# qcc4cp/qcc

Hardware: AMD Instinct MI355X
Metric: gate-applies/sec (2^30-amplitude units), QFT (higher is better)
Workload: dtype f64; 1 GPU; 30-qubit QFT complex128, 465 gates/step (qc.qft order), basis-state input, state resident in HBM, 2^30 amplitudes per GPU [BASELINE config 2]; qubits=30, fusion=1

## Files before the change

include/qcc_hip.h:

```cpp
#ifndef QCC_HIP_H_
#define QCC_HIP_H_

#include <stdint.h>

#ifdef __cplusplus
extern "C" {
#endif

typedef struct qh_state_s *qh_handle;

#define QH_OK 0
#define QH_ERR_BAD_QUBIT 1
#define QH_ERR_SAME_QUBIT 2
#define QH_ERR_BAD_DTYPE 3
#define QH_ERR_HIP 4
#define QH_ERR_ARG 5
#define QH_ERR_NOMEM 6
#define QH_ERR_NO_DEVICE 7
#define QH_ERR_NONLOCAL 8
#define QH_ERR_COMM 9

#define QH_FUSE_OFF 0
#define QH_FUSE_SWEEP 1

// ... 80 lines not shown
int qh_comm_destroy(qh_handle h);
int qh_exchange_alltoall(qh_handle h, int base_bit, uint64_t chunk_amps);
int qh_exchange_pair(qh_handle h, int shard_bit, int local_bit, uint64_t chunk_amps);
int qh_exchange_loopback(qh_handle h, int local_bit, uint64_t chunk_amps);
int qh_exchange_wait(qh_handle h);
int qh_exchange_stats(qh_handle h, qh_xstats *out);
int qh_comm_allreduce_sum(qh_handle h, double *inout, int count);

int qh_norm2(qh_handle h, double *out);
int qh_amplitude(qh_handle h, uint64_t logical_index, double out[2]);
int qh_argmax(qh_handle h, uint64_t *phys_index, double *prob);
int qh_prob_bit(qh_handle h, int logical_bit, double *p1);
int qh_prob_bit_value(qh_handle h, int logical_bit, int value, double *p);
int qh_scale(qh_handle h, double re, double im);
int qh_project_bit(qh_handle h, int logical_bit, int value);
int qh_marginal(qh_handle h, int k, const int32_t *bits, double *out);
int qh_sample(qh_handle h, uint64_t count, const double *u, uint64_t *logical_out);
int qh_project_bits(qh_handle h, uint64_t mask, uint64_t value);
int qh_expect_pauli(qh_handle h, uint64_t nterms, const uint64_t *xmask, const uint64_t *zmask, double *out);
typedef struct { uint64_t index; double re, im; } qh_entry;
#define QH_SELECT_MAX (1u << 20)
#define QH_TOPK_MAX 4096
int qh_select(qh_handle h, double threshold, uint64_t cap, qh_entry *out, uint64_t *count, double *weight);
int qh_topk(qh_handle h, uint64_t k, qh_entry *out, uint64_t *count);
int qh_amplitudes(qh_handle h, uint64_t count, const uint64_t *logical, double *out, uint64_t *nlocal);

int qh_clone(qh_handle src, qh_handle *out);
int qh_copy(qh_handle dst, qh_handle src);
int qh_inner(qh_handle a, qh_handle b, double out[2]);
#define QH_INNER_LINEAR 0
#define QH_INNER_TILES 1
#define QH_INNER_GATHER 2
typedef struct {
  uint32_t path;
  uint32_t nrest;
  uint64_t free_a, free_b;
  uint8_t tile_a[8], tile_b[8], shuffle[8];
  uint8_t rest_a[56], rest_b[56];
  uint8_t pos_b[64];
} qh_inner_tiles;
int qh_inner_plan(qh_handle a, qh_handle b, qh_inner_tiles *out);
int qh_axpby(qh_handle dst, const double alpha[2], qh_handle src, const double beta[2], double *norm2);

int qh_extend(qh_handle src, int k, const double *amps, uint64_t basis, qh_handle *out);
int qh_release(qh_handle src, int k, const int32_t *bits, uint64_t value, double weight[2], qh_handle *out);

typedef struct {
  uint64_t gates_submitted;
  uint64_t kernels_launched;
  uint64_t sweeps;
  uint64_t bytes_algorithmic;
  uint64_t bytes_swept;
  uint64_t gates_noop;
} qh_stats;
int qh_get_stats(qh_handle h, qh_stats *out);
int qh_reset_stats(qh_handle h);
int qh_timer_begin(qh_handle h);
int qh_timer_end(qh_handle h, float *milliseconds);
int qh_timer_lap(qh_handle h);
int qh_timer_laps(qh_handle h, float *milliseconds, int cap, int *count);
int qh_plan_json(qh_handle h, char *buf, uint64_t cap, uint64_t *needed);

int qh_plan_export(qh_handle h, void *buf, uint64_t cap, uint64_t *needed);

int qh_plan_handlers(qh_handle h, void *buf, uint64_t cap, uint64_t *needed);

int qh_host_apply1(void *psi, const double gate[8], int nbits, int tgt,
                   int bit_width);
int qh_host_applyc(void *psi, const double gate[8], int nbits, int ctl, int tgt,
                   int bit_width);
int qh_host_release(void);

#ifdef __cplusplus
}
#endif
#endif
```

qcc_amd/csrc/engine.hip:

```cpp
#include <hip/hip_runtime.h>

#include <algorithm>
#include <chrono>
#include <cmath>
#include <cstdarg>
#include <cstddef>
#include <cstdio>
#include <cstdlib>
#include <cstring>
#include <ctime>
#include <string>
#include <vector>

#include "../../include/qcc_hip.h"
#include "buffers.hip.h"
#include "kernels_gate.hip.h"
#include "kernels_dense.hip.h"
#include "kernels_mux.hip.h"
#include "kernels_measure.hip.h"
#include "kernels_select.hip.h"
#include "select_plan.h"
#include "kernels_expect.hip.h"
#include "kernels_inner.hip.h"
#include "kernels_axpby.hip.h"
// ... 2393 lines not shown
                    (uint32_t)__builtin_popcountll(xmask[t] & zmask[t]) & 3u};
  }
  std::stable_sort(terms.begin(), terms.end(), [](const Term &l, const Term &r) { return l.px < r.px; });
  qh::ScratchLayout lay;
  const size_t slab_off = lay.add((size_t)kExpectBlocks * qh::kExpectT * sizeof(double)), out_off = lay.add((size_t)nterms * sizeof(double));
  HIP_TRY(h->meas.reserve(lay.total));
  double *slab = (double *)(h->meas.as<char>() + slab_off), *dout = (double *)(h->meas.as<char>() + out_off);
  uint64_t batches = 0;
  for (uint64_t first = 0; first < nterms;) {
    uint64_t cnt = 1;
    while (first + cnt < nterms && cnt < (uint64_t)qh::kExpectT && terms[first + cnt].px == terms[first].px) ++cnt;
    const uint64_t px = terms[first].px;
    const bool pair = (px >> 6) != 0;
    qh::ExpectArgs a{};
    a.x = px;
    a.tb = pair ? 63 - __builtin_clzll(px) : 0;
    const int per_bits = pair ? 3 : 4, nom = 8 + per_bits, wbits = pair ? h->nloc - 1 : h->nloc;
    a.cw = std::min(nom, wbits);
    const uint64_t nchunks = 1ull << (wbits - a.cw), nblk = std::min(nchunks, kExpectBlocks);
    a.cpb = (uint32_t)(nchunks / nblk);
    for (uint64_t k = 0; k < cnt; ++k) {
      const Term &tm = terms[first + k];
      uint64_t z = tm.pz;
      if (pair) z = (z & ((1ull << a.tb) - 1ull)) | ((z >> (a.tb + 1)) << a.tb);
      a.zt[k] = (uint8_t)(z & 255ull);
      const uint32_t zu = (uint32_t)(z >> 8) & ((1u << per_bits) - 1u);
      for (uint32_t u = 0; u < (1u << per_bits); ++u) a.zu[k] |= (uint16_t)((__builtin_popcount(u & zu) & 1) << u);
      a.zc[k] = z >> nom;
      const uint32_t one = (((tm.ny >> 1) ^ tm.neg) & 1u) ? 0xBFF00000u : 0x3FF00000u;
      if (tm.ny & 1u) a.cim[k] = one; else a.cre[k] = one;
    }
    const int tt = cnt <= 4 ? 4 : qh::kExpectT;
    with_real(h, [&](auto x) {
      using R = decltype(x);
      if (tt == 4) launch_expect<R, 4>(h, pair, (unsigned)nblk, a, slab);
      else launch_expect<R, qh::kExpectT>(h, pair, (unsigned)nblk, a, slab);
    });
    hipLaunchKernelGGL(qh::k_expect_fold, dim3((unsigned)cnt), dim3(256), 0, h->stream, (const double *)slab, (uint32_t)nblk, tt,
                       pair ? 2.0 : 1.0, dout + first);
    if ((rc = check_launch(h))) return rc;
    first += cnt;
    ++batches;
  }
  std::vector<double> vals(nterms);
  if ((rc = read_back(h, vals.data(), dout, (size_t)nterms * sizeof(double)))) return rc;
  for (uint64_t k = 0; k < nterms; ++k) out[terms[k].idx] = vals[k];
  h->stats.kernels_launched += batches;
  h->stats.bytes_swept += batches * ((1ull << h->nloc) * h->amp_bytes());
  return QH_OK;
}

int qh_get_stats(qh_handle h, qh_stats *out) {
  if (!h || !out) return fail(QH_ERR_ARG, "null");
  *out = h->stats;
  return QH_OK;
}
int qh_reset_stats(qh_handle h) {
  if (!h) return fail(QH_ERR_ARG, "null");
  h->stats = qh_stats{};
  return QH_OK;
}

int qh_timer_begin(qh_handle h) {
  if (!h) return fail(QH_ERR_ARG, "null handle");
  int rc = enter(h);
  if (rc) return rc;
  rc = make_events(h);
  if (rc) return rc;
  HIP_TRY(hipEventRecord(h->ev0, h->stream));
  return QH_OK;
}
int qh_timer_end(qh_handle h, float *ms) {
  if (!h || !ms) return fail(QH_ERR_ARG, "null handle or out");
  if (!h->ev0) return fail(QH_ERR_ARG, "qh_timer_end without qh_timer_begin");
  int rc = enter(h);
  if (rc) return rc;
  HIP_TRY(hipEventRecord(h->ev1, h->stream));
  if ((rc = wait_event(h, h->ev1, "qh_timer_end"))) return rc;
  HIP_TRY(hipEventElapsedTime(ms, h->ev0, h->ev1));
  return QH_OK;
}

int qh_timer_lap(qh_handle h) {
  if (!h) return fail(QH_ERR_ARG, "null handle");
  const int rc = enter(h);
  if (rc) return rc;
  if (h->laps_used == h->laps.size()) {
    hipEvent_t e = nullptr;
    HIP_TRY(hipEventCreate(&e));
    h->laps.push_back(e);
  }
  HIP_TRY(hipEventRecord(h->laps[h->laps_used++], h->stream));
  return QH_OK;
}
int qh_timer_laps(qh_handle h, float *ms, int cap, int *count) {
  if (!h || !count || h->dry) return fail(QH_ERR_ARG, "null/dry");
  HIP_TRY(hipSetDevice(h->device));
  const int n = h->laps_used > 0 ? (int)h->laps_used - 1 : 0;
  if (h->laps_used) {
    const int rc = wait_event(h, h->laps[h->laps_used - 1], "qh_timer_laps");
    if (rc) return rc;
  }
  for (int k = 0; k < n && ms && k < cap; ++k) HIP_TRY(hipEventElapsedTime(&ms[k], h->laps[k], h->laps[k + 1]));
  *count = n;
  h->laps_used = 0;
  return QH_OK;
// ... 647 lines not shown
```

qcc_amd/csrc/kernels_sweep.hip.h:

```cpp
#pragma once
#include <hip/hip_runtime.h>

#include <string>
#include <vector>

#include "kernels_gate.hip.h"
#include <deque>
#include <memory>

#include "planner.h"
#include "exchange.hip.h"

namespace qh {

struct SweepParams {
  const SweepOp *ops;
  const DGroup *groups;
  const OTerm *oterms;
  uint32_t nops;
  uint32_t tables_rel;
  uint32_t n_ltab_lds;
  uint32_t pad0;
  uint64_t store_delta_mask;
  uint64_t prof_buf;
  uint64_t tilemax;
  uint64_t slot_off[64];
  uint64_t slot_off_store[64];
};
static_assert(kMaxInsertBits + kMaxSlabBits <= kMaxIns, "planner/kernels disagree on inserted bits");
static_assert(kExchangeSlabBits == kMaxSlabBits, "exchange_plan.h / planner disagree on slab bits");
static_assert(sizeof(SweepOp) == 96 && sizeof(DGroup) == 64 && sizeof(OTerm) == 24, "asm island layouts");
static_assert(offsetof(SweepParams, slot_off) == 0x40 && offsetof(SweepParams, nops) == 0x18 && offsetof(SweepParams, tilemax) == 0x38 &&
                  offsetof(SweepParams, slot_off_store) == 0x240 && offsetof(SweepParams, store_delta_mask) == 0x28,
              "asm island layouts");

struct LaneGeom {
  int lane_low;
  int rot;
  int blk_bits;
  int nwave;
  int wpos[kMaxWaveBits];
  int wdst[kMaxWaveBits];
  int ltab_in_island;
};

constexpr uint64_t kProfRows = 8192, kProfRecs = 128;
struct UnitPerm {
  int n;
  int shift[kMaxUnitSegs];
  uint64_t mask[kMaxUnitSegs];
  int nslab;
  int slab_pos[kMaxSlabBits];
  uint64_t slab_val;
};

struct alignas(8) SweepArgs {
  uint64_t psi;
  uint64_t dst;
  uint64_t prm;
  uint64_t idx_high;
  uint64_t nunits;
  uint64_t ins_ones;
  uint64_t slab_val;
  uint64_t ltab_src;
  uint32_t n_ltab;
  uint32_t exch_bytes;
  uint32_t stride_units;
  uint32_t seat_dest;
  uint8_t ins_n, lane_low, rot, blk_bits;
  uint8_t nwave, wpos[2], island_copies;
  uint8_t wdst[2], up_n, up_nslab;
  uint8_t slab_pos[kMaxSlabBits], wpb;
  uint8_t seat[8];
  uint8_t ins_pos[16];
  int8_t up_shift[kMaxUnitSegs];
  uint64_t up_mask[kMaxUnitSegs];
};
static_assert(kMaxUnitSegs == 8 && kMaxSlabBits == 3 && kMaxIns <= 16 && kMaxWaveBits == 2 && kLaneBits <= 8, "SweepArgs layout");
static_assert(offsetof(SweepArgs, n_ltab) == 64 && offsetof(SweepArgs, ins_n) == 80 && offsetof(SweepArgs, ins_pos) == 104 &&
                  offsetof(SweepArgs, up_shift) == 120 && offsetof(SweepArgs, up_mask) == 128 && sizeof(SweepArgs) == 192,
              "SweepArgs layout (k_sweep reads it by dword index)");

typedef uint32_t qh_u32x16 __attribute__((ext_vector_type(16)));

inline int flush_pace(const PlanResult &pr, bool wide, int nloc) {
  if (const char *e = getenv("QH_SWEEP_PACE")) return atoi(e);
  if (!wide || pr.sweeps.empty()) return 0;
  double joules = 0, ms = 0;
  for (const SweepPlan &sp : pr.sweeps) {
    if (sp.nwave > 1) return 0;
    const double units = (double)sp.swept_bytes / (2.0 * 16.0 * (double)(1ull << 30));
    ms += (nloc <= 31 ? 5.45 : 5.85) * units;
    joules += 4.9 * units + sweep_op_energy_nj(sp) * (double)sp.ntiles * 1e-9 * 1.15;
  }
  const double watts = joules / ms * 1e3;
  return (watts >= 1320.0 && watts <= 1450.0) ? 12 : 0;
}

template <int RB, bool WIDE>
__global__ __launch_bounds__(256) void k_sweep(SweepArgs args_in_kernarg_segment) {
  constexpr uint32_t kAmp = WIDE ? 16u : 8u;
#ifdef QH_PROF
  const uint64_t prof_t_entry = __builtin_amdgcn_s_memtime();
#endif
  const uint32_t lane_u = threadIdx.x & 63;
  const uint32_t wave_s = __builtin_amdgcn_readfirstlane(threadIdx.x >> 6);
  extern __shared__ __attribute__((aligned(16))) unsigned char xbuf[];
  const uint32_t lds_base = (uint32_t)(uintptr_t)(__attribute__((address_space(3))) unsigned char *)xbuf;
  for (uint32_t turn = 0;; ++turn) {
    qh_u32x16 q0, q1, q2;
    asm volatile("s_load_dwordx16 %0, %3, 0x0\n\ts_load_dwordx16 %1, %3, 0x40\n\ts_load_dwordx16 %2, %3, 0x80\n\t"
                 "s_waitcnt lgkmcnt(0)"
                 : "=&s"(q0), "=&s"(q1), "=&s"(q2)
                 : "s"((uint64_t)(uintptr_t)__builtin_amdgcn_kernarg_segment_ptr()));
    auto dw = [&](int i) -> uint32_t { return i < 16 ? q0[i] : i < 32 ? q1[i - 16] : q2[i - 32]; };
    auto qw = [&](int i) -> uint64_t { return (uint64_t)dw(i) | ((uint64_t)dw(i + 1) << 32); };
    auto by = [&](int i, int b) -> uint32_t { return (dw(i) >> (8 * b)) & 255u; };
    const uint32_t lane_low = by(20, 1), nwave = by(21, 0), wpb = by(23, 3);
    const uint32_t n_lt = dw(16), exch_bytes = dw(17);
    const uint32_t lds_ltab = lds_base + exch_bytes;
    const uint32_t wg_threads = wpb << 6;
    const bool island_copies = by(21, 3) != 0;
    if (turn == 0 && n_lt && !island_copies) {
      typedef double v2d_t __attribute__((ext_vector_type(2)));
      const __attribute__((address_space(1))) v2d_t *src = (const __attribute__((address_space(1))) v2d_t *)qw(14);
      v2d_t *dst = (v2d_t *)(xbuf + exch_bytes);
      for (uint32_t i = threadIdx.x; i < n_lt * 64u; i += wg_threads) dst[i] = src[i];
      __syncthreads();
    }
    const uint32_t nlt_now = island_copies && turn == 0 ? n_lt : 0u;
    uint64_t bi = blockIdx.x;
    const uint32_t rot = by(20, 2), blk_bits = by(20, 3);
    if (rot) bi = ((bi >> rot) | (bi << (blk_bits - rot))) & ((1ull << blk_bits) - 1);
    const uint32_t upb = wpb >> nwave;
    const uint64_t wu = bi * upb + (wave_s >> nwave) + (uint64_t)turn * dw(18);
    if (wu >= qw(8)) break;
    uint32_t lane_t = lane_u;
    asm volatile("" : "+v"(lane_t));
    uint32_t loff = 0;
#pragma unroll
    for (int i = 0; i < kLaneBits; ++i) loff |= ((lane_t >> i) & 1u) << by(24 + i / 4, i % 4);
    const uint32_t voff = loff * kAmp;
    uint64_t wave_off = 0, woff = 0;
#pragma unroll
    for (int j = 0; j < kMaxWaveBits; ++j)
      if ((uint32_t)j < nwave) {
        wave_off |= (uint64_t)((wave_s >> j) & 1u) << by(21, 1 + j);
        woff |= (uint64_t)((wave_s >> j) & 1u) << by(22, j);
      }
// ... 146 lines not shown
  for (size_t k = 0; k < sp.ops.size(); ++k) {
    SweepOp *o = ops_out + k;
    if ((o->kind & 0xffffu) != OP_DIAG) continue;
    bool any = false, all_neg = true;
    for (uint32_t gi = 0; gi < o->n_groups; ++gi) {
      const DGroup &g = sp.groups[o->group_off + gi];
      if (g.reg_mask) continue;
      any = true;
      all_neg &= !(g.flags & (DG_LTAB | DG_BITFAC)) && !g.ntab && !g.n_oterms && g.re == -1.0 && g.im == 0.0;
    }
    if (any && all_neg) o->flags |= 1u << 9;
  }
  if (bw == 128)
    for (size_t k = 0; k < sp.ops.size(); ++k) {
      SweepOp *o = ops_out + k;
      if ((o->kind & 0xffffu) != OP_DIAG || o->n_groups != 1 || (o->flags & OPF_DEFER_C)) continue;
      const DGroup &g = sp.groups[o->group_off];
      if (!g.reg_mask || (g.flags & (DG_LTAB | DG_BITFAC)) || g.ntab || g.n_oterms || g.lane_mask > 63u) continue;
      const uint32_t cls = (g.re == -1.0 && g.im == 0.0) ? 0u : g.lane_mask == 0 ? 1u : 2u;
      const uint32_t mi = reg_mask_number(g.reg_mask, sp.rb);
      o->kind = OP_DIAG | ((kHidDiag1 + 16u * cls + mi) << 16);
      o->tb = g.lane_mask | (g.reg_mask << 8);
      memcpy(&o->cm_reg, &g.re, 8);
      memcpy(&o->cm_thread, &g.im, 8);
    }
  if (!sp.groups.empty()) memcpy(groups_out, sp.groups.data(), sp.groups.size() * sizeof(DGroup));
  for (size_t k = 0; k < sp.groups.size(); ++k) {
    DGroup *g = groups_out + k;
    if (n_ltab_lds && (g->flags & DG_LTAB) && g->ltab_off / 64 < n_ltab_lds) g->flags |= DG_LTAB_LDS;
    bool sign_ot = !(g->flags & (DG_LTAB | DG_BITFAC)) && g->ntab == 0 && g->n_oterms > 0 && g->re == 1.0 && g->im == 0.0;
    for (uint32_t t = 0; sign_ot && t < g->n_oterms; ++t) {
      const OTerm &o = sp.oterms[g->oterm_off + t];
      sign_ot = o.re == -1.0 && o.im == 0.0;
    }
    g->flags |= group_handler_bits(*g, sp.rb, sign_ot);
  }
}

struct PlanCacheEntry {
  std::vector<GateRec> queue;
  std::string key;
  std::shared_ptr<const PlanResult> plan;
};

inline bool same_queue(const std::vector<GateRec> &a, const std::vector<GateRec> &b) {
  if (a.size() != b.size()) return false;
  for (size_t i = 0; i < a.size(); ++i)
    if (a[i].ctl_mask != b[i].ctl_mask || a[i].tgt != b[i].tgt || a[i].neg_mask != b[i].neg_mask ||
        memcmp(a[i].g, b[i].g, sizeof a[i].g) != 0)
      return false;
  return true;
}

struct SweepBuffers {
  std::deque<PlanCacheEntry> plans;
  StagedUpload<1> ops;
};

inline bool sweep_supported(int nloc, int bw) { return (bw == 128 || bw == 64) && nloc >= kLaneBits + 2; }

template <bool WIDE> inline void sweep_block_shape(const SweepPlan &sp, int *wpb, size_t *exch_bytes) {
  const bool contiguous = sp.contiguous();
  *wpb = contiguous ? 2 : 4;
  *exch_bytes = 0;
  if (sp.nwave) {
    *wpb = 1 << sp.nwave;
    const int nr = 1 << sp.rb;
    *exch_bytes = (size_t)*wpb * std::min(8, nr / 2) * 64 * (WIDE ? 16 : 8);
  }
}

template <bool WIDE> inline int ltab_lds_count(const SweepPlan &sp) {
  constexpr int cap = 16;
  int wpb;
  size_t exch;
  sweep_block_shape<WIDE>(sp, &wpb, &exch);
  const long per_wg = 160l * 1024 * wpb / 12 - (long)exch - 512;
  const int fit = (int)std::max(0l, per_wg / 1024);
  return std::max(0, std::min(std::min(sp.n_ltab, cap), fit));
}

inline int sweep_rot(bool contiguous) { return contiguous ? 3 : 6; }

inline uint64_t sweep_tile_bits(const SweepPlan &sp) {
  uint64_t m = ((1ull << sp.lane_low) - 1) | sp.fixed_ones;
  for (int k = 0; k < sp.rb; ++k) m |= (1ull << sp.regpos[k]) | (1ull << sp.regpos_store[k]);
  for (int k = 0; k < sp.nlanehi(); ++k) m |= 1ull << sp.lanehi[k];
  for (int k = 0; k < sp.nwave; ++k) m |= 1ull << sp.wavepos[k];
  return m;
}

inline bool sweep_takes_slab(const SweepPlan &sp, uint64_t slab_mask) {
  return !(sweep_tile_bits(sp) & slab_mask) && popc(slab_mask) <= kMaxSlabBits &&
         popc(sp.fixed_ones) + sp.rb + sp.nlanehi() + sp.nwave + popc(slab_mask) <= kMaxIns &&
         (sp.ntiles >> popc(slab_mask)) >= 64;
}

inline BitIns make_tile_ins(const SweepPlan &sp, uint64_t slab_mask = 0, uint64_t slab_val = 0) {
  BitIns ins{};
  ins.n = 0;
  ins.ones = sp.fixed_ones | slab_val;
  uint64_t regmask = slab_mask;
  for (int k = 0; k < sp.rb; ++k) regmask |= 1ull << sp.regpos[k];
  for (int k = 0; k < sp.nlanehi(); ++k) regmask |= 1ull << sp.lanehi[k];
  for (int k = 0; k < sp.nwave; ++k) regmask |= 1ull << sp.wavepos[k];
  for (int b = 0; b < 64; ++b)
    if (((regmask | sp.fixed_ones) >> b) & 1ull) ins.pos[ins.n++] = b;
  return ins;
}
// ... 89 lines not shown
                         void *dst) {
  if (bw == 128) launch_sweep_t<true>(sp, psi, nloc, shard, stream, d_prm, h_prm, pace, slab_mask, slab_val, dst);
  else launch_sweep_t<false>(sp, psi, nloc, shard, stream, d_prm, h_prm, pace, slab_mask, slab_val, dst);
}

struct TileMaxOut {
  void *buf = nullptr;
  uint64_t cap = 0;
  bool valid = false;
  uint64_t nunits = 0;
  BitIns ins{};
  uint64_t tile_mask = 0;
};

struct SlabIO {
  std::vector<Arrival> *arrivals = nullptr;
  bool split_last = false;
  uint64_t avoid = 0;
  int want_bits = 3;
  Comm *comm = nullptr;
  uint64_t slab_mask = 0;
  std::vector<uint64_t> slab_vals;
  std::vector<hipEvent_t> slab_done;
  bool split_done = false;
  uint64_t sweeps_overlapped = 0;
};

inline void wait_all_arrivals(std::vector<Arrival> *arr, hipStream_t stream) {
  if (!arr) return;
  for (const Arrival &a : *arr) if (a.ev) (void)hipStreamWaitEvent(stream, a.ev, 0);
  arr->clear();
}

inline int run_fused(const std::vector<GateRec> &queue, const PlanRequest &rq, void *psi, hipStream_t stream, bool dry,
                     SweepBuffers *bufs, qh_stats *stats, std::string *err, SlabIO *slab = nullptr, void *psi_alt = nullptr,
                     void **result = nullptr, uint8_t *final_pos = nullptr, TileMaxOut *tmax = nullptr) {
  const int nloc = rq.nloc, bw = rq.bw;
  const uint64_t shard = rq.shard;
  std::shared_ptr<const PlanResult> cached;
  const int rc = guard_planning(err, [&] {
    const std::string key = rq.key();
    const bool use_cache = !getenv("QH_PLAN_CACHE") || atoi(getenv("QH_PLAN_CACHE")) != 0;
    if (use_cache)
      for (auto &e : bufs->plans)
        if (e.key == key && same_queue(e.queue, queue)) { cached = e.plan; return; }
    cached = std::make_shared<const PlanResult>(plan_best(queue, rq));
    if (use_cache) {
      bufs->plans.push_front(PlanCacheEntry{queue, key, cached});
      if (bufs->plans.size() > 4) bufs->plans.pop_back();
    }
  });
  if (rc) return rc;
  const PlanResult &pr = *cached;
  const int pace = dry ? 0 : flush_pace(pr, bw == 128, nloc);
  stats->gates_noop += pr.noop_gates;
  size_t n_ops = 0, n_groups = 0, n_ot = 0, n_tab = 0;
  for (auto &sp : pr.sweeps) {
    if (popc(sp.fixed_ones) + sp.rb + sp.nlanehi() + sp.nwave > kMaxIns) {
      *err = "sweep needs more inserted bits than the tile enumeration supports";
      return QH_ERR_ARG;
    }
    n_ops += sp.ops.size() + 1;
    n_groups += sp.groups.size();
    n_ot += sp.oterms.size();
    n_tab += sp.tables.size();
  }
  const bool want_tmax = tmax && tmax->buf && !dry && !slab && !pr.sweeps.empty() && pr.sweeps.back().fixed_ones == 0 &&
                         (pr.sweeps.back().ntiles >> pr.sweeps.back().nwave) <= tmax->cap;
  if (tmax) tmax->valid = false;
  const size_t bytes_prm = pr.sweeps.size() * sizeof(SweepParams);
  const size_t bytes_ops = n_ops * sizeof(SweepOp), bytes_groups = n_groups * sizeof(DGroup),
               bytes_ot = (n_ot * sizeof(OTerm) + 15) / 16 * 16, bytes_tab = n_tab * sizeof(double);
  const size_t total = bytes_prm + bytes_ops + bytes_groups + bytes_ot + bytes_tab + 256;
  std::vector<char> host_dry;
  char *hbase = nullptr, *d_base = nullptr;
  if (dry) {
    host_dry.resize(total);
    hbase = host_dry.data();
  } else {
    if (hipEvent_t e = bufs->ops.busy()) (void)hipEventSynchronize(e);
    size_t cap = bufs->ops.host.cap;
    if (cap < total) {
      if (cap) (void)hipStreamSynchronize(stream);
      cap = std::max<size_t>(total * 2, 1 << 20);
    }
    unsigned slot = 0;
    const hipError_t e = bufs->ops.acquire(cap, &hbase, &d_base, &slot);
    if (e != hipSuccess) {
      *err = std::string("op buffers (pinned + device): ") + hipGetErrorString(e);
      return e == hipErrorOutOfMemory ? QH_ERR_NOMEM : QH_ERR_HIP;
    }
  }
  memset(hbase, 0, total);
  char *h_prm = hbase, *h_ops = h_prm + bytes_prm, *h_groups = h_ops + bytes_ops,
       *h_ot = h_groups + bytes_groups, *h_tab = h_ot + bytes_ot;
  {
    size_t io = 0, ig = 0, it = 0, is = 0, itab = 0;
    for (auto &sp : pr.sweeps) {
      SweepParams prm{};
      prm.ops = (const SweepOp *)(d_base + bytes_prm) + io;
      prm.groups = (const DGroup *)(d_base + bytes_prm + bytes_ops) + ig;
      prm.oterms = (const OTerm *)(d_base + bytes_prm + bytes_ops + bytes_groups) + it;
      prm.nops = (uint32_t)sp.ops.size();
      prm.n_ltab_lds = (uint32_t)(bw == 128 ? ltab_lds_count<true>(sp) : ltab_lds_count<false>(sp));
      prm.tables_rel = (uint32_t)((d_base + bytes_prm + bytes_ops + bytes_groups + bytes_ot + itab * sizeof(double)) -
                                  (const char *)prm.groups);
      for (int k = 0; k < 64; ++k) {
        uint64_t o = 0;
        for (int b = 0; b < sp.rb; ++b)
          if ((k >> b) & 1) o |= 1ull << sp.regpos[b];
        prm.slot_off[k] = o * (bw == 128 ? 16 : 8);
        o = 0;
        for (int b = 0; b < sp.rb; ++b)
          if ((k >> b) & 1) o |= 1ull << (sp.relayout ? sp.reg_dest[b] : sp.regpos_store[b]);
        prm.slot_off_store[k] = o * (bw == 128 ? 16 : 8);
      }
      prm.store_delta_mask = sp.relayout ? 0ull : ~0ull;
      if (want_tmax && is + 1 == pr.sweeps.size()) prm.tilemax = (uint64_t)tmax->buf;
      memcpy(h_prm + is * sizeof(SweepParams), &prm, sizeof prm);
      build_device_copy(sp, bw, prm.n_ltab_lds, (SweepOp *)(h_ops + io * sizeof(SweepOp)), (DGroup *)(h_groups + ig * sizeof(DGroup)));
      if (!sp.oterms.empty()) memcpy(h_ot + it * sizeof(OTerm), sp.oterms.data(), sp.oterms.size() * sizeof(OTerm));
      if (!sp.tables.empty()) memcpy(h_tab + itab * sizeof(double), sp.tables.data(), sp.tables.size() * sizeof(double));
      io += sp.ops.size() + 1; ig += sp.groups.size(); it += sp.oterms.size(); itab += sp.tables.size(); is++;
    }
  }
  if (!dry) {
    hipError_t e = hipMemcpyAsync(d_base, hbase, total, hipMemcpyHostToDevice, stream);
    if (e == hipSuccess) e = bufs->ops.commit(stream, 0);
    if (e != hipSuccess) {
      *err = std::string("hipMemcpyAsync(op buffer): ") + hipGetErrorString(e);
      return QH_ERR_HIP;
    }
  }
#ifdef QH_PROF
  static char *d_prof = nullptr;
  const size_t prof_bytes = kProfRows * kProfRecs * 8;
  if (!dry) {
    if (!d_prof) (void)hipMalloc(&d_prof, prof_bytes * 16);
    (void)hipMemsetAsync(d_prof, 0, prof_bytes * 16, stream);
    for (size_t k = 0; k < pr.sweeps.size() && k < 16; ++k) {
      const uint64_t v = (uint64_t)(d_prof + k * prof_bytes);
      (void)hipMemcpyAsync(d_base + k * sizeof(SweepParams) + offsetof(SweepParams, prof_buf), &v, 8,
                           hipMemcpyHostToDevice, stream);
      (void)hipStreamSynchronize(stream);
    }
  }
#endif
  if (result) *result = psi;
  if (final_pos) memcpy(final_pos, pr.final_pos, 64);
  static const bool timing = env_flag("QH_SWEEP_TIMING", false);
  std::vector<hipEvent_t> tev;
  void *cur = psi, *other = psi_alt;
  size_t is = 0;
  uint64_t avoid_cur = slab ? slab->avoid : 0;
  uint64_t earlier_tiles = 0;
  for (auto &sp : pr.sweeps) {
    auto moved = [&](uint64_t v) {
      if (!sp.relayout) return v;
      uint64_t o = v >> nloc << nloc;
      for (uint64_t t = v & ((1ull << nloc) - 1); t; t &= t - 1) o |= 1ull << sp.dest_pos[__builtin_ctzll(t)];
      return o;
    };
    if (sp.relayout && !dry && !other) {
      *err = "internal: a relayout sweep was planned without a second buffer";
      return QH_ERR_ARG;
    }
    const SweepParams *prm = (const SweepParams *)d_base + is;
    SweepParams hprm;
    memcpy(&hprm, h_prm + is * sizeof(SweepParams), sizeof hprm);
    const bool first = is == 0, last = is + 1 == pr.sweeps.size();
    bool launched = false;
    if (slab) {
      if (first && slab->arrivals && !slab->arrivals->empty()) {
        const uint64_t am = (*slab->arrivals)[0].slab_mask;
        const bool split_too = last && slab->split_last;
        if (am && !split_too && sweep_takes_slab(sp, am)) {
          for (const Arrival &a : *slab->arrivals) {
            if (dry) continue;
            (void)hipStreamWaitEvent(stream, a.ev, 0);
            launch_sweep(sp, cur, nloc, shard, bw, stream, prm, hprm, pace, a.slab_mask, a.slab_val, sp.relayout ? other : nullptr);
          }
          slab->arrivals->clear();
          slab->sweeps_overlapped++;
          launched = true;
        } else {
          wait_all_arrivals(slab->arrivals, stream);
        }
      }
      if (!launched && last && slab->split_last && (slab->comm || dry)) {
        const int want = std::min(slab->want_bits, kMaxSlabBits);
        const uint64_t taken_bits = avoid_cur | sweep_tile_bits(sp);
        uint64_t m = pick_slab_bits(nloc, taken_bits | ~earlier_tiles, want, kLaneBits);
        if (popc(m) < want) m |= pick_slab_bits(nloc, taken_bits | m, want - popc(m), kLaneBits);
        while (m && !sweep_takes_slab(sp, m)) m &= m - 1;
        if (m) {
          const int K = 1 << popc(m);
          for (int k = 0; k < K; ++k) {
            const uint64_t sv = deposit_bits((uint64_t)k, m);
            hipEvent_t e = nullptr;
            if (!dry) {
              launch_sweep(sp, cur, nloc, shard, bw, stream, prm, hprm, pace, m, sv, sp.relayout ? other : nullptr);
              e = slab->comm->event();
              if (e) (void)hipEventRecord(e, stream);
            }
            slab->slab_done.push_back(e);
            slab->slab_vals.push_back(moved(sv));
          }
          slab->slab_mask = moved(m);
          slab->sweeps_overlapped++;
          slab->split_done = true;
          launched = true;
        }
      }
    }
    if (timing && !dry) {
      hipEvent_t e;
      (void)hipEventCreate(&e);
      (void)hipEventRecord(e, stream);
      tev.push_back(e);
    }
    if (want_tmax && last) {
      tmax->nunits = sp.ntiles >> sp.nwave;
      if (hipMemsetAsync(tmax->buf, 0, tmax->nunits * 8, stream) != hipSuccess) { *err = "hipMemsetAsync(tile maxima)"; return QH_ERR_HIP; }
      uint64_t tm = 0;
      const int tb = kLaneBits + sp.rb + sp.nwave;
      if (sp.relayout) tm = (1ull << tb) - 1;
      else {
        for (int i = 0; i < kLaneBits; ++i) tm |= 1ull << sp.seat_store[i];
        for (int k = 0; k < sp.rb; ++k) tm |= 1ull << sp.regpos_store[k];
        for (int k = 0; k < sp.nwave; ++k) tm |= 1ull << sp.wavepos_store[k];
      }
      tmax->tile_mask = tm;
      tmax->ins = BitIns{};
      for (int b = 0; b < 64; ++b) if ((tm >> b) & 1ull) tmax->ins.pos[tmax->ins.n++] = b;
      tmax->valid = popc(tm) == tb && tmax->ins.n <= kMaxIns;
    }
    if (!dry && !launched) launch_sweep(sp, cur, nloc, shard, bw, stream, prm, hprm, pace, 0, 0, sp.relayout ? other : nullptr);
    if (!dry && sp.relayout) {
      std::swap(cur, other);
      if (result) *result = cur;
    }
    avoid_cur = moved(avoid_cur);
    earlier_tiles = moved(earlier_tiles | (sweep_tile_bits(sp) & ~((1ull << kLaneBits) - 1)));
    is++;
    stats->kernels_launched++;
    stats->sweeps++;
    stats->bytes_algorithmic += sp.alg_bytes;
    stats->bytes_swept += sp.swept_bytes;
  }
#ifdef QH_PROF
  if (!dry && getenv("QH_PROF_OUT")) {
    (void)hipStreamSynchronize(stream);
    std::vector<uint64_t> rec(kProfRows * kProfRecs);
    FILE *f = fopen(getenv("QH_PROF_OUT"), "a");
    for (size_t k = 0; f && k < pr.sweeps.size() && k < 16; ++k) {
      const SweepPlan &sp = pr.sweeps[k];
      (void)hipMemcpy(rec.data(), d_prof + k * prof_bytes, prof_bytes, hipMemcpyDeviceToHost);
      const size_t nrec = std::min<size_t>(sp.ops.size() + 5, kProfRecs);
      std::vector<std::vector<double>> dt(nrec);
      size_t rows = 0;
      for (size_t r = 0; r < kProfRows; ++r) {
        const uint64_t *t = &rec[r * kProfRecs];
        if (!t[0] || !t[nrec - 1]) continue;
        rows++;
        for (size_t j = 0; j + 1 < nrec; ++j) dt[j].push_back((double)(t[j + 1] - t[j]));
      }
      double life = 0, real = 0, tmin = 1e300, tmax = 0, rmin = 1e300, rmax = 0;
      for (size_t r = 0; r < kProfRows; ++r) {
        const uint64_t *t = &rec[r * kProfRecs];
        if (!t[0] || !t[nrec - 1] || !t[126] || !t[127]) continue;
        life += (double)(t[nrec - 1] - t[0]);
        real += (double)(t[127] - t[126]);
        tmin = std::min(tmin, (double)t[0]); tmax = std::max(tmax, (double)t[nrec - 1]);
        rmin = std::min(rmin, (double)t[126]); rmax = std::max(rmax, (double)t[127]);
      }
      fprintf(f, "sweep %zu rb %d nwave %d relayout %d ops %zu rows %zu\n", k, sp.rb, sp.nwave, (int)sp.relayout, sp.ops.size(), rows);
      if (real > 0)
        fprintf(f, "  s_memtime ticks per 10 ns of s_memrealtime: %.3f (waves), %.3f (whole sweep); sweep = %.3f ms by the 100 MHz counter; "
                   "mean wave lifetime %.0f ticks\n", life / real, (tmax - tmin) / (rmax - rmin), (rmax - rmin) * 1e-5, life / rows);
      auto stat = [&](size_t j, const char *what) {
        std::vector<double> &v = dt[j];
        if (v.empty()) return;
        std::sort(v.begin(), v.end());
        double sum = 0;
        for (double x : v) sum += x;
        fprintf(f, "  %-44s mean %9.0f  p10 %8.0f  median %8.0f  p90 %8.0f\n", what, sum / v.size(), v[v.size() / 10], v[v.size() / 2],
                v[v.size() * 9 / 10]);
      };
      stat(0, "tile load (issue + wait)");
      char what[128];
      for (size_t j = 0; j < sp.ops.size() && j + 2 < nrec - 1; ++j) {
        const SweepOp &o = sp.ops[j];
        static const char *kn[] = {"REG", "LANE", "DIAG", "LSWAP", "WSWAP"};
        snprintf(what, sizeof what, "op %2zu %-5s tb %u flags %#x groups %u", j, kn[o.kind], o.tb, o.flags, o.kind == OP_DIAG ? o.n_groups : 0);
        stat(j + 2, what);
      }
      stat(1, "first op header wait / dispatch");
      {
        std::vector<double> v;
        for (size_t r = 0; r < kProfRows; ++r) {
          const uint64_t *t = &rec[r * kProfRecs];
          if (t[0] && t[125] && t[0] > t[125]) v.push_back((double)(t[0] - t[125]));
// ... 37 lines not shown
```

qcc_amd/native.py:

```python
import ctypes
import os
import subprocess

PKG = os.path.dirname(os.path.abspath(__file__))
ROOT = os.path.dirname(PKG)
LIB_PATH = os.environ.get('QCC_HIP_LIB') or os.path.join(PKG, 'libqcc_hip.so')
SOURCES = [os.path.join(PKG, 'csrc', f) for f in
           ('engine.hip', 'buffers.hip.h', 'kernels_gate.hip.h', 'kernels_dense.hip.h', 'kernels_mux.hip.h', 'kernels_measure.hip.h', 'kernels_select.hip.h', 'select_plan.h', 'kernels_expect.hip.h', 'kernels_inner.hip.h', 'kernels_axpby.hip.h', 'inner_plan.h', 'kernels_resize.hip.h', 'resize_plan.h', 'kernels_sweep.hip.h', 'planner.h', 'exchange.hip.h', 'exchange_plan.h',
            'sweep_island_rb2.inc', 'sweep_island_rb3.inc', 'sweep_island_rb4.inc',
            'sweep_island_rb5.inc', 'sweep_island_f32_rb2.inc', 'sweep_island_f32_rb3.inc',
            'sweep_island_f32_rb4.inc', 'sweep_island_f32_rb5.inc', 'sweep_island_f32_rb6.inc', 'sweep_handlers.inc',
            'libq_facade.cc')]
HEADERS = [os.path.join(ROOT, 'include', 'libq.h')]
HEADER = os.path.join(ROOT, 'include', 'qcc_hip.h')

QH_OK = 0
QH_ERR_BAD_QUBIT, QH_ERR_SAME_QUBIT, QH_ERR_BAD_DTYPE, QH_ERR_HIP = 1, 2, 3, 4
QH_ERR_ARG, QH_ERR_NOMEM, QH_ERR_NO_DEVICE, QH_ERR_NONLOCAL, QH_ERR_COMM = 5, 6, 7, 8, 9
QH_FUSE_OFF, QH_FUSE_SWEEP = 0, 1

_u64, _i32, _vp, _dp = ctypes.c_uint64, ctypes.c_int, ctypes.c_void_p, ctypes.POINTER(ctypes.c_double)


class QhStats(ctypes.Structure):
  _fields_ = [('gates_submitted', _u64), ('kernels_launched', _u64), ('sweeps', _u64),
              ('bytes_algorithmic', _u64), ('bytes_swept', _u64), ('gates_noop', _u64)]

  def as_dict(self):
    return {k: int(getattr(self, k)) for k, _ in self._fields_}


QH_INNER_LINEAR, QH_INNER_TILES, QH_INNER_GATHER = 0, 1, 2


class QhInnerTiles(ctypes.Structure):
  _u8 = ctypes.c_uint8
  _fields_ = [('path', ctypes.c_uint32), ('nrest', ctypes.c_uint32), ('free_a', _u64), ('free_b', _u64),
              ('tile_a', _u8 * 8), ('tile_b', _u8 * 8), ('shuffle', _u8 * 8), ('rest_a', _u8 * 56), ('rest_b', _u8 * 56),
              ('pos_b', _u8 * 64)]

  def as_dict(self):
    return {k: (int(getattr(self, k)) if isinstance(getattr(self, k), int) else list(getattr(self, k))) for k, _ in self._fields_}


QH_SELECT_MAX, QH_TOPK_MAX = 1 << 20, 4096


class QhEntry(ctypes.Structure):
  _fields_ = [('index', _u64), ('re', ctypes.c_double), ('im', ctypes.c_double)]


SIGNATURES = {
    'qh_last_error': (ctypes.c_char_p, []),
    'qh_version': (_i32, []),
    'qh_device_count': (_i32, [ctypes.POINTER(_i32)]),
    'qh_create': (_i32, [_i32, _i32, _i32, ctypes.POINTER(_vp)]),
    'qh_attach': (_i32, [_i32, _i32, _i32, _vp, _vp, ctypes.POINTER(_vp)]),
    'qh_create_dry': (_i32, [_i32, _i32, ctypes.POINTER(_vp)]),
    'qh_create_host_mapped': (_i32, [_i32, _i32, _i32, ctypes.POINTER(_vp)]),
    'qh_host_ptr': (_i32, [_vp, ctypes.POINTER(_vp)]),
    'qh_destroy': (_i32, [_vp]),
    'qh_set_shard': (_i32, [_vp, _i32, _u64]),
    'qh_device_ptr': (_i32, [_vp, ctypes.POINTER(_vp)]),
    'qh_stream': (_i32, [_vp, ctypes.POINTER(_vp)]),
    'qh_nbits': (_i32, [_vp, ctypes.POINTER(_i32), ctypes.POINTER(_i32)]),
    'qh_init_basis': (_i32, [_vp, _u64]),
    'qh_init_product': (_i32, [_vp, _i32, ctypes.POINTER(_i32), ctypes.POINTER(_vp), ctypes.POINTER(_u64)]),
    'qh_upload': (_i32, [_vp, _vp, _u64, _u64]),
    'qh_download': (_i32, [_vp, _vp, _u64, _u64]),
    'qh_apply1': (_i32, [_vp, _i32, _dp]),
    'qh_applyc': (_i32, [_vp, _i32, _i32, _dp]),
    'qh_apply_bits': (_i32, [_vp, _u64, _i32, _dp]),
    'qh_apply_matrix': (_i32, [_vp, _i32, ctypes.POINTER(ctypes.c_int32), _u64, _dp]),
    'qh_apply_mux': (_i32, [_vp, _i32, ctypes.POINTER(ctypes.c_int32), _i32, _dp]),
    'qh_apply_diag': (_i32, [_vp, _i32, ctypes.POINTER(ctypes.c_int32), _dp]),
    'qh_set_fusion': (_i32, [_vp, _i32]),
    'qh_set_relayout': (_i32, [_vp, _i32, ctypes.POINTER(_i32)]),
    'qh_apply_stream': (_i32, [_vp, _u64, ctypes.POINTER(ctypes.c_int32), _dp]),
    'qh_flush': (_i32, [_vp]),
# ... 137 lines not shown
```

Measured before the change: 28400 gate-applies/s.

## Add adaptive feedback controller for sweep pacing based on measured flush times

Replaces the static power-model pace choice with a per-plan feedback controller. Each flush is timed with HIP events, and the controller moves the pace up a ladder when a flush runs much slower than the best seen, treating that as clock throttling. It also probes lower pace values after long clean stretches. The aim is to avoid power or clock clamping on the wide single-GPU path while keeping pacing overhead small, at the cost of event records per flush and possible oscillation between pace levels.

```diff
diff --git a/include/qcc_hip.h b/include/qcc_hip.h
--- a/include/qcc_hip.h
+++ b/include/qcc_hip.h
@@ -156,6 +156,8 @@
   uint64_t bytes_algorithmic;
   uint64_t bytes_swept;
   uint64_t gates_noop;
+  uint64_t sweep_pace;
+  uint64_t flushes_clamped;
 } qh_stats;
 int qh_get_stats(qh_handle h, qh_stats *out);
 int qh_reset_stats(qh_handle h);
diff --git a/qcc_amd/csrc/engine.hip b/qcc_amd/csrc/engine.hip
--- a/qcc_amd/csrc/engine.hip
+++ b/qcc_amd/csrc/engine.hip
@@ -2469,6 +2469,7 @@
 
 int qh_get_stats(qh_handle h, qh_stats *out) {
   if (!h || !out) return fail(QH_ERR_ARG, "null");
+  if (!h->dry && use_device(h) == QH_OK) h->stats.flushes_clamped += h->sweep.pace.poll();
   *out = h->stats;
   return QH_OK;
 }
diff --git a/qcc_amd/csrc/kernels_sweep.hip.h b/qcc_amd/csrc/kernels_sweep.hip.h
--- a/qcc_amd/csrc/kernels_sweep.hip.h
+++ b/qcc_amd/csrc/kernels_sweep.hip.h
@@ -10,6 +10,7 @@
 
 #include "planner.h"
 #include "exchange.hip.h"
+#include "pace_control.h"
 
 namespace qh {
 
@@ -83,8 +84,7 @@
 
 typedef uint32_t qh_u32x16 __attribute__((ext_vector_type(16)));
 
-inline int flush_pace(const PlanResult &pr, bool wide, int nloc) {
-  if (const char *e = getenv("QH_SWEEP_PACE")) return atoi(e);
+inline int flush_pace_model(const PlanResult &pr, bool wide, int nloc) {
   if (!wide || pr.sweeps.empty()) return 0;
   double joules = 0, ms = 0;
   for (const SweepPlan &sp : pr.sweeps) {
@@ -95,6 +95,25 @@
   }
   const double watts = joules / ms * 1e3;
   return (watts >= 1320.0 && watts <= 1450.0) ? 12 : 0;
+}
+
+inline PaceSwitches pace_switches() {
+  PaceSwitches sw;
+  if (const char *e = getenv("QH_SWEEP_PACE")) { sw.pinned = true; sw.pin = atoi(e); }
+  if (const char *e = getenv("QH_PACE_ADAPT")) sw.adapt = atoi(e) != 0;
+  return sw;
+}
+
+inline uint64_t pace_plan_key(const PlanResult &pr, int bw, int nloc) {
+  uint64_t h = 1469598103934665603ull;
+  auto mix = [&](uint64_t v) { for (int i = 0; i < 8; ++i) { h ^= (v >> (8 * i)) & 255u; h *= 1099511628211ull; } };
+  mix((uint64_t)bw << 8 | (uint64_t)nloc);
+  for (const SweepPlan &sp : pr.sweeps) {
+    mix(sp.swept_bytes);
+    mix((uint64_t)sp.rb | (uint64_t)sp.nwave << 8 | (uint64_t)sp.relayout << 16);
+    mix((uint64_t)(sweep_op_energy_nj(sp) + 0.5));
+  }
+  return h;
 }
 
 template <int RB, bool WIDE>
@@ -347,9 +366,61 @@
   return true;
 }
 
+struct PaceLoop {
+  static constexpr int kPairs = 4;
+  struct Pair {
+    hipEvent_t t0 = nullptr, t1 = nullptr;
+    uint64_t key = 0;
+    int pace = 0;
+  } pair[kPairs];
+  unsigned head = 0, pending = 0;
+  PaceController ctl;
+  PaceLoop() = default;
+  PaceLoop(const PaceLoop &) = delete;
+  PaceLoop &operator=(const PaceLoop &) = delete;
+  ~PaceLoop() {
+    for (Pair &p : pair) {
+      if (p.t0) (void)hipEventDestroy(p.t0);
+      if (p.t1) (void)hipEventDestroy(p.t1);
+    }
+  }
+  uint64_t poll() {
+    uint64_t clamped = 0;
+    while (pending) {
+      Pair &p = pair[head % kPairs];
+      const hipError_t q = hipEventQuery(p.t1);
+      if (q == hipErrorNotReady) {
+        (void)hipGetLastError();
+        break;
+      }
+      float ms = 0;
+      if (q == hipSuccess && hipEventElapsedTime(&ms, p.t0, p.t1) == hipSuccess) clamped += ctl.observe(p.key, p.pace, (double)ms);
+      else (void)hipGetLastError();
+      head++;
+      pending--;
+    }
+    return clamped;
+  }
+  Pair *begin(uint64_t key, int pace, hipStream_t stream) {
+    if (pending == kPairs) return nullptr;
+    Pair &p = pair[(head + pending) % kPairs];
+    if (!p.t0 && hipEventCreate(&p.t0) != hipSuccess) { p.t0 = nullptr; (void)hipGetLastError(); return nullptr; }
+    if (!p.t1 && hipEventCreate(&p.t1) != hipSuccess) { p.t1 = nullptr; (void)hipGetLastError(); return nullptr; }
+    if (hipEventRecord(p.t0, stream) != hipSuccess) { (void)hipGetLastError(); return nullptr; }
+    p.key = key;
+    p.pace = pace;
+    return &p;
+  }
+  void end(Pair *p, hipStream_t stream) {
+    if (hipEventRecord(p->t1, stream) == hipSuccess) pending++;
+    else (void)hipGetLastError();
+  }
+};
+
 struct SweepBuffers {
   std::deque<PlanCacheEntry> plans;
   StagedUpload<1> ops;
+  PaceLoop pace;
 };
 
 inline bool sweep_supported(int nloc, int bw) { return (bw == 128 || bw == 64) && nloc >= kLaneBits + 2; }
@@ -545,7 +616,15 @@
   });
   if (rc) return rc;
   const PlanResult &pr = *cached;
-  const int pace = dry ? 0 : flush_pace(pr, bw == 128, nloc);
+  const PaceSwitches psw = pace_switches();
+  const bool multi_rank = slab && slab->comm && slab->comm->nranks > 1;
+  int pace = psw.pinned ? psw.pin : multi_rank ? 0 : flush_pace_model(pr, bw == 128, nloc);
+  bool adapt = !dry && !slab && !psw.pinned && psw.adapt && bw == 128 && !pr.sweeps.empty();
+  for (const SweepPlan &sp : pr.sweeps) adapt = adapt && sp.nwave <= 1;
+#ifdef QH_PROF
+  adapt = false;
+#endif
+  const uint64_t pace_key = adapt ? pace_plan_key(pr, bw, nloc) : 0;
   stats->gates_noop += pr.noop_gates;
   size_t n_ops = 0, n_groups = 0, n_ot = 0, n_tab = 0;
   for (auto &sp : pr.sweeps) {
@@ -572,6 +651,8 @@
     hbase = host_dry.data();
   } else {
     if (hipEvent_t e = bufs->ops.busy()) (void)hipEventSynchronize(e);
+    stats->flushes_clamped += bufs->pace.poll();
+    if (adapt) pace = bufs->pace.ctl.next(pace_key, pace);
     size_t cap = bufs->ops.host.cap;
     if (cap < total) {
       if (cap) (void)hipStreamSynchronize(stream);
@@ -645,6 +726,8 @@
   std::vector<hipEvent_t> tev;
   void *cur = psi, *other = psi_alt;
   size_t is = 0;
+  stats->sweep_pace = (uint64_t)std::max(0, std::min(255, pace));
+  PaceLoop::Pair *pace_pair = adapt ? bufs->pace.begin(pace_key, pace, stream) : nullptr;
   uint64_t avoid_cur = slab ? slab->avoid : 0;
   uint64_t earlier_tiles = 0;
   for (auto &sp : pr.sweeps) {
@@ -741,6 +824,7 @@
     stats->bytes_algorithmic += sp.alg_bytes;
     stats->bytes_swept += sp.swept_bytes;
   }
+  if (pace_pair) bufs->pace.end(pace_pair, stream);
 #ifdef QH_PROF
   if (!dry && getenv("QH_PROF_OUT")) {
     (void)hipStreamSynchronize(stream);
diff --git a/qcc_amd/csrc/pace_control.h b/qcc_amd/csrc/pace_control.h
--- /dev/null
+++ b/qcc_amd/csrc/pace_control.h
@@ -0,0 +1,152 @@
+#pragma once
+#include <stdint.h>
+
+namespace qh {
+
+constexpr int kPaceLadder[] = {0, 4, 8, 12, 16, 24};
+constexpr int kPaceRungs = (int)(sizeof kPaceLadder / sizeof kPaceLadder[0]);
+constexpr double kPaceClampRatio = 1.03;
+constexpr double kPaceSpread = 0.005;
+constexpr int kPaceWindow = 8;
+constexpr int kPaceClampsToAct = 2;
+constexpr int kPaceCleanToDescend = 32;
+constexpr int kPaceSettle = 2;
+constexpr int kPaceReprobeWindows = 64;
+constexpr int kPaceReprobeMax = 4096;
+constexpr int kPacePlans = 4;
+
+inline int pace_rung_at_least(int pace) {
+  for (int r = 0; r < kPaceRungs; ++r)
+    if (kPaceLadder[r] >= pace) return r;
+  return kPaceRungs - 1;
+}
+
+struct PacePlanState {
+  uint64_t key = 0;
+  bool used = false;
+  uint64_t stamp = 0;
+  int rung = 0;
+  int floor = 0;
+  double best = 0;
+  int seen = 0;
+  int n = 0, clamps = 0;
+  double sum = 0;
+  bool trial = false;
+  bool probing = false;
+  double ref_mean = 0;
+  int quiet = 0;
+  int clean = 0;
+  int failed_rung = -1;
+  int reprobe_after = kPaceReprobeWindows;
+  uint64_t clamped_flushes = 0;
+};
+
+class PaceController {
+ public:
+  int next(uint64_t key, int model_pace) {
+    PacePlanState *s = find(key);
+    if (!s) {
+      s = &plans_[victim()];
+      *s = PacePlanState{};
+      s->key = key;
+      s->used = true;
+      s->rung = pace_rung_at_least(model_pace < 0 ? 0 : model_pace);
+    }
+    s->stamp = ++clock_;
+    last_ = s;
+    return kPaceLadder[s->rung];
+  }
+
+  bool observe(uint64_t key, int pace, double ms) {
+    PacePlanState *s = find(key);
+    if (!s || !(ms > 0) || pace != kPaceLadder[s->rung]) return false;
+    if (s->seen < kPaceSettle) {
+      s->seen++;
+      return false;
+    }
+    const bool clamp = s->best > 0 && ms > s->best * kPaceClampRatio;
+    if (s->best == 0 || ms < s->best) s->best = ms;
+    s->n++;
+    s->sum += ms;
+    s->clean = clamp ? 0 : s->clean < kPaceCleanToDescend ? s->clean + 1 : s->clean;
+    if (clamp) {
+      s->clamps++;
+      s->clamped_flushes++;
+      total_clamped_++;
+    }
+    if (s->clamps >= (s->trial ? 1 : kPaceClampsToAct)) close_window(s, true);
+    else if (s->n >= kPaceWindow) close_window(s, false);
+    return clamp;
+  }
+
+  int current_pace() const { return last_ ? kPaceLadder[last_->rung] : 0; }
+  uint64_t clamped_flushes() const { return total_clamped_; }
+  const PacePlanState *state(uint64_t key) const { return const_cast<PaceController *>(this)->find(key); }
+
+ private:
+  PacePlanState plans_[kPacePlans];
+  PacePlanState *last_ = nullptr;
+  uint64_t clock_ = 0, total_clamped_ = 0;
+
+  PacePlanState *find(uint64_t key) {
+    for (PacePlanState &p : plans_)
+      if (p.used && p.key == key) return &p;
+    return nullptr;
+  }
+  int victim() const {
+    int v = 0;
+    for (int i = 0; i < kPacePlans; ++i) {
+      if (!plans_[i].used) return i;
+      if (plans_[i].stamp < plans_[v].stamp) v = i;
+    }
+    return v;
+  }
+  static void new_window(PacePlanState *s) {
+    s->n = s->clamps = 0;
+    s->sum = 0;
+  }
+  static void step_up(PacePlanState *s) {
+    if (s->rung <= s->failed_rung) s->reprobe_after = s->reprobe_after * 2 > kPaceReprobeMax ? kPaceReprobeMax : s->reprobe_after * 2;
+    else s->failed_rung = s->rung;
+    const int up = s->rung + 1 < kPaceRungs ? s->rung + 1 : kPaceRungs - 1;
+    s->floor = s->rung = up;
+    s->quiet = 0;
+    s->trial = s->probing = false;
+  }
+  static void close_window(PacePlanState *s, bool clamped) {
+    const double mean = s->sum / (double)s->n;
+    new_window(s);
+    if (clamped) {
+      step_up(s);
+      return;
+    }
+    if (s->trial) {
+      if (mean > s->ref_mean * (1.0 + kPaceSpread)) {
+        step_up(s);
+        return;
+      }
+      if (s->probing) {
+        s->floor = s->rung;
+        s->quiet = 0;
+      }
+      s->trial = s->probing = false;
+    } else {
+      s->quiet++;
+    }
+    if (s->rung == 0 || s->clean < kPaceCleanToDescend) return;
+    const bool below_floor = s->rung - 1 < s->floor;
+    if (below_floor && s->quiet < s->reprobe_after) return;
+    s->ref_mean = mean;
+    s->rung--;
+    s->trial = true;
+    s->probing = below_floor;
+  }
+};
+
+struct PaceSwitches {
+  bool pinned = false;
+  int pin = 0;
+  bool adapt = true;
+};
+
+}
diff --git a/qcc_amd/native.py b/qcc_amd/native.py
--- a/qcc_amd/native.py
+++ b/qcc_amd/native.py
@@ -6,7 +6,7 @@
 ROOT = os.path.dirname(PKG)
 LIB_PATH = os.environ.get('QCC_HIP_LIB') or os.path.join(PKG, 'libqcc_hip.so')
 SOURCES = [os.path.join(PKG, 'csrc', f) for f in
-           ('engine.hip', 'buffers.hip.h', 'kernels_gate.hip.h', 'kernels_dense.hip.h', 'kernels_mux.hip.h', 'kernels_measure.hip.h', 'kernels_select.hip.h', 'select_plan.h', 'kernels_expect.hip.h', 'kernels_inner.hip.h', 'kernels_axpby.hip.h', 'inner_plan.h', 'kernels_resize.hip.h', 'resize_plan.h', 'kernels_sweep.hip.h', 'planner.h', 'exchange.hip.h', 'exchange_plan.h',
+           ('engine.hip', 'buffers.hip.h', 'kernels_gate.hip.h', 'kernels_dense.hip.h', 'kernels_mux.hip.h', 'kernels_measure.hip.h', 'kernels_select.hip.h', 'select_plan.h', 'kernels_expect.hip.h', 'kernels_inner.hip.h', 'kernels_axpby.hip.h', 'inner_plan.h', 'kernels_resize.hip.h', 'resize_plan.h', 'kernels_sweep.hip.h', 'planner.h', 'exchange.hip.h', 'exchange_plan.h', 'pace_control.h',
             'sweep_island_rb2.inc', 'sweep_island_rb3.inc', 'sweep_island_rb4.inc',
             'sweep_island_rb5.inc', 'sweep_island_f32_rb2.inc', 'sweep_island_f32_rb3.inc',
             'sweep_island_f32_rb4.inc', 'sweep_island_f32_rb5.inc', 'sweep_island_f32_rb6.inc', 'sweep_handlers.inc',
@@ -24,7 +24,8 @@
 
 class QhStats(ctypes.Structure):
   _fields_ = [('gates_submitted', _u64), ('kernels_launched', _u64), ('sweeps', _u64),
-              ('bytes_algorithmic', _u64), ('bytes_swept', _u64), ('gates_noop', _u64)]
+              ('bytes_algorithmic', _u64), ('bytes_swept', _u64), ('gates_noop', _u64),
+              ('sweep_pace', _u64), ('flushes_clamped', _u64)]
 
   def as_dict(self):
     return {k: int(getattr(self, k)) for k, _ in self._fields_}
```

After: 28360 gate-applies/s. No clear change (-0.1%).
